# lightest/cellularautomatons3d

Hardware: AMD Instinct MI355X
Metric: Gcells/s CA step at 512^3 (higher is better)
Workload: dtype u32

## Files before the change

cellularautomatons3d_amd/csrc/ca3d_api.cpp:

```cpp
#include <cstdarg>
#include <cstdio>
#include <cstring>
#include <cstdlib>
#include <new>
#include <stdexcept>

#include "ca3d_engine.h"

namespace
{
thread_local char g_last_error[1024] = "";
}

namespace ca3d
{
void set_last_error(const char *msg) noexcept
{
	if (!msg) msg = "";
	size_t n = strlen(msg);
	if (n >= sizeof g_last_error) n = sizeof g_last_error - 1;
	memmove(g_last_error, msg, n);
	g_last_error[n] = 0;
}

// ... 846 lines not shown
			}
			if (cur == h->cur) break;
		}
		return CA3D_OK;
	}
	if (!strcmp(name, "stats")) { h->want_stats = value ? 1 : 0; if (!value) h->ev_valid = false; return CA3D_OK; }
	if (!strcmp(name, "graph_min"))
	{
		if (value < 1 || value > kMaxGraphSteps) return fail(CA3D_ERR_INVALID_ARGUMENT, "graph_min must be in [1, %u]", kMaxGraphSteps);
		h->graph_min = (uint32_t)value;
		return CA3D_OK;
	}
	if (!strcmp(name, "render_indirect")) { h->render_indirect = value ? 1 : 0; return CA3D_OK; }
	if (!strcmp(name, "render_sched")) { h->render_sched = value ? 1 : 0; return CA3D_OK; }
	if (!strcmp(name, "render_skip")) { h->render_skip = value ? 1 : 0; return CA3D_OK; }
	if (!strcmp(name, "rows"))
	{
		h->use_rows = value ? 1 : 0;
		refresh_kernels(h);
		return CA3D_OK;
	}
	if (!strcmp(name, "render_frame_bricks")) { h->render_frame_bricks = value ? 1 : 0; return CA3D_OK; }
	if (!strcmp(name, "render_stream")) { h->render_stream = value ? 1 : 0; return CA3D_OK; }
	if (!strcmp(name, "render_pipeline"))
	{
		if (value < 0 || value > ca3d_engine::kMaxLanes) return fail(CA3D_ERR_INVALID_ARGUMENT, "render_pipeline must be 0 (off), 1 (default depth) or 2 .. %d frames in flight", ca3d_engine::kMaxLanes);
		h->render_pipeline = (int)value;
		return CA3D_OK;
	}
	if (!strcmp(name, "render_stream_check")) { h->render_stream_check = value ? 1 : 0; return CA3D_OK; }
	if (!strcmp(name, "render_row_begin") || !strcmp(name, "render_row_end"))
	{
		if (value < 0 || value > 16384) return fail(CA3D_ERR_INVALID_ARGUMENT, "row %lld is outside any target", (long long)value);
		if (name[11] == 'b')
		{
			if (value % 16) return fail(CA3D_ERR_INVALID_ARGUMENT, "render_row_begin must be a multiple of 16 (the renderer's tile height)");
			h->render_row0 = (uint32_t)value;
		}
		else h->render_row1 = (uint32_t)value;
		return CA3D_OK;
	}
	if (!strcmp(name, "render_mode"))
	{
		if (value != 0 && value != 1) return fail(CA3D_ERR_INVALID_ARGUMENT, "render_mode must be 0 (converged frame) or 1 (one literal reference frame)");
		h->render_mode = (int)value;
		return CA3D_OK;
	}
	if (!strcmp(name, "render_reset_history"))
	{
		int rc2 = bind_device(h);
		if (rc2) return rc2;
		return clear_render_history(h);
	}
	if (!strcmp(name, "fused")) { drop_graph(h); h->use_fused = value ? 1 : 0; return CA3D_OK; }
	if (!strcmp(name, "variant"))
	{
		if (value != 0 && value != 1) return fail(CA3D_ERR_INVALID_ARGUMENT, "variant must be 0 (auto) or 1 (generic kernel)");
		drop_graph(h);
		h->variant = (int)value;
		refresh_kernels(h);
		return CA3D_OK;
	}
	if (!strcmp(name, "resident"))
	{
		h->use_resident = value ? 1 : 0;
		if (value) h->res_failed = false;
		refresh_kernels(h);
		return CA3D_OK;
	}
	if (!strcmp(name, "resident_rows"))
	{
		if (value != 16 && value != 32) return fail(CA3D_ERR_INVALID_ARGUMENT, "resident_rows must be 16 or 32");
		if ((uint32_t)value != h->res_rows)
		{
			int rc2 = bind_device(h);
			if (rc2) return rc2;
			HIP_TRY(hipStreamSynchronize(h->stream));
			free_resident(h);
			h->res_rows = (uint32_t)value;
			refresh_kernels(h);
		}
		return CA3D_OK;
	}
	if (!strcmp(name, "resident_pair"))
	{
		if (value != 0 && value != 1) return fail(CA3D_ERR_INVALID_ARGUMENT, "resident_pair must be 0 or 1");
		if ((value != 0) != h->res_pair)
		{
			int rc2 = bind_device(h);
			if (rc2) return rc2;
			HIP_TRY(hipStreamSynchronize(h->stream));
			free_resident(h);
			h->res_pair = value != 0;
			refresh_kernels(h);
		}
		return CA3D_OK;
	}
	if (!strcmp(name, "resident_zsplit"))
	{
		if (value != 1 && value != 2) return fail(CA3D_ERR_INVALID_ARGUMENT, "resident_zsplit must be 1 or 2");
		h->res_zsplit = (uint32_t)value;
		refresh_kernels(h);
		return CA3D_OK;
	}
	if (!strcmp(name, "resident_min"))
	{
		if (value < 1) return fail(CA3D_ERR_INVALID_ARGUMENT, "resident_min must be >= 1");
// ... 70 lines not shown
```

cellularautomatons3d_amd/csrc/ca3d_engine.h:

```cpp
#pragma once

#include <map>
#include <string>
#include <vector>

#include "ca3d_internal.h"

struct ca3d_engine
{
	int device = 0;
	hipStream_t own_stream = nullptr;
	hipStream_t stream = nullptr;
	hipEvent_t ev_start = nullptr, ev_stop = nullptr;
	bool ev_valid = false;

	bool configured = false;
	uint32_t G = 0;
	int layout = CA3D_LAYOUT_PACKED32;
	bool slab = false;
	uint32_t z0 = 0, nz = 0, ghost = 0;
	uint32_t nplanes = 0;
	size_t plane_words = 0;
	uint32_t *buf[2] = {nullptr, nullptr};
	bool has_state = false;
	bool binary_state = false;
	uint64_t step = 0;
	uint32_t cur = 0;

	ca3d::CanonRules rules;
	int variant = 0;
	int use_graph = 1;
	int render_mode = 0;
	int render_indirect = 0;
	int render_sched = 1;
	uint32_t render_row0 = 0, render_row1 = 0;
	int use_fused = 0;

	struct StepGraph { hipGraphExec_t exec = nullptr; uint32_t launches = 0; };
	std::map<uint64_t, StepGraph> step_graphs;
	uint32_t graph_min = 128;
	int want_stats = 1;
	std::map<uint64_t, hipGraphExec_t> slab_graphs;
	uint32_t pending_edges = 0;
	bool pending_binary = true;
	bool pending_resident = false;
	int roll_z = 0;
	int roll_tile = 1;
	int use_roll = 1;
	int use_jit = 1;
	ca3d::VnJit vn_jit;
	ca3d::ClassJit class_jit;
	ca3d::RowsJit rows_jit;
	int use_rows = 1;
	ca3d::RollJit roll_jit;
	std::string jit_log;

	int use_resident = 1;
	bool res_ready = false;
	bool res_class = false;
	bool res_failed = false;
	bool res_check = false;
	void *res_jit_fn = nullptr;
	void *res_slab_fn = nullptr;
	size_t res_mail_bytes = 0;
	unsigned long long *res_mail = nullptr;
	uint32_t *res_status = nullptr, *res_status_host = nullptr;
	uint32_t res_epoch = 0;
	uint32_t res_min = 8;
	uint32_t queue_max = 0;
	uint32_t queued = 0;
	uint64_t launches_total = 0;
	bool res_pair = true;
	uint32_t res_rows = 32;
	uint32_t res_zsplit = 1;
	uint32_t res_timeout_ticks = 20000000;
	uint32_t *spare = nullptr;
	struct ResPending { uint32_t epoch0, n, cur_before; uint64_t step_before; uint32_t *in, *other, *spare; };
	std::vector<ResPending> res_pending;
	uint32_t res_fault_tile = 0;
	uint32_t res_recovered = 0;
	std::string res_note;

	void *comm = nullptr;
	int comm_rank = 0, comm_world = 0;
	hipStream_t comm_stream = nullptr;
	hipEvent_t ev_edges = nullptr, ev_comm = nullptr, ev_gather = nullptr;
	bool ghosts_valid = false;

	ca3d_stats stats{};
// ... 130 lines not shown
```

cellularautomatons3d_amd/csrc/ca3d_internal.h:

```cpp
#pragma once

#include <hip/hip_runtime.h>
#include <stdint.h>
#include <string>

#include "ca3d.h"
#include "ca_device_types.h"

namespace ca3d
{

constexpr int kMaxOffsets = 26;

struct OffsetLists
{
	uint32_t n[3];
	uint8_t code[3][32];
};

struct CanonRules
{
	bool valid = false;
	MainKind main = MAIN_GENERIC;
	bool need[3] = {false, false, false};
	bool fast = false;
	OffsetLists lists{};
	PackedRuleArgs prog{};
	uint32_t onset_survive[3]{}, onset_born[3]{};
	uint32_t unpacked_survive = 0, unpacked_born = 0;
	RuleSetProg unpacked_prog{};
	bool unpacked_fast = false;
	uint32_t survive_raw[CA3D_LUT_LEN]{}, born_raw[CA3D_LUT_LEN]{};
};

int canonicalize_rules(const int32_t *main_offs, uint32_t n_main, const int32_t *edge_offs, uint32_t n_edge,
                       const int32_t *corner_offs, uint32_t n_corner, const uint32_t *survive,
                       const uint32_t *born, CanonRules *out, std::string *err);
void compile_rule_prog(uint32_t onset_mask, uint32_t max_count, RuleProg *out);


struct VnJit
{
	void *zr1 = nullptr, *zr2 = nullptr, *zr4 = nullptr, *zr8 = nullptr;
	int cvl = -1;
	uint32_t lut_s = 0, lut_b = 0;
};

struct RowsJit
{
	void *deep = nullptr, *flat = nullptr;
	uint32_t G = 0;
	int zrun = 0, main = -1;
	bool e = false, c = false;
};

struct ClassJit
{
	void *deep = nullptr, *deep_za = nullptr, *flat = nullptr;
	void *deep_np2 = nullptr, *flat_np2 = nullptr;
	int main = -1;
	bool e = false, c = false;
};

struct RollJit
{
	void *z[3] = {nullptr, nullptr, nullptr};
	void *tile[4] = {nullptr, nullptr, nullptr, nullptr};
	void *tile_x = nullptr; int zx = 0;
	void *loop[2][2] = {{nullptr, nullptr}, {nullptr, nullptr}};
	void *w2[2] = {nullptr, nullptr};
	void *wtile[2] = {nullptr, nullptr};
	void *np2[3] = {nullptr, nullptr, nullptr};
	int cv_np2 = 0;
	int cvl = -1;
	int main = -1;
	bool e = false, c = false;
};

struct PackedLaunch
{
	const uint32_t *in;
	uint32_t *out;
	PlaneRange pr;
	const CanonRules *rules;
	int variant;
	const VnJit *vn_jit = nullptr;
	const ClassJit *class_jit = nullptr;
	const RollJit *roll_jit = nullptr;
	int roll_z = 0;
	int roll_tile = 1;
	const RowsJit *rows_jit = nullptr;
};

struct ResidentLaunch
{
// ... 147 lines not shown
	int neighbourhood;
	bool clustered;
	uint32_t first, count;
	const uint32_t *periods;
	ca3d_canon_period *out;
	uint64_t *keys;
	uint32_t keys_stride;
};
hipError_t launch_canon_period(const CanonPeriodLaunch &l, hipStream_t stream);
struct SheetLaunch
{
	const uint32_t *state;
	uint32_t first, count;
	uint32_t tile_w, tile_h, columns, spp;
	const float *uniforms;
	uint32_t *presentation;
	void *light;
	uint32_t *depth;
	unsigned long long *counters;
};
hipError_t launch_render_sheet(const SheetLaunch &l, hipStream_t stream);
uint32_t sheet_shares(uint32_t count, uint32_t blocks, uint32_t slots);
struct SeedLaunch
{
	uint32_t *buf0, *buf1;
	uint32_t G;
	int layout;
	uint32_t z0, nz, ghost;
	ca3d_seed spec;
};
hipError_t launch_seed(const SeedLaunch &l, hipStream_t stream);
hipError_t launch_seed_ensemble(uint32_t *state, uint32_t *prev, uint32_t first, uint32_t count, const ca3d_seed *specs, const ca3d_seed &one, hipStream_t stream);
const char *seed_spec_error(const ca3d_seed &s, uint32_t G);
hipError_t launch_copy_f4(const void *in, void *out, size_t bytes, hipStream_t stream);
hipError_t streams_concurrent(hipStream_t a, hipStream_t b, bool *out);
hipError_t launch_render(const RenderLaunch &l, hipStream_t stream);
size_t stream_scratch_bytes(uint32_t W, uint32_t H, uint32_t spp, size_t *hit_off, size_t *occl_off, size_t *rays_off);
size_t frame_bricks_bytes(uint32_t G);
bool frame_bricks_applies(uint32_t G);
hipError_t launch_render_frame_bricks(const void *frame_params, uint32_t *bricks, bool bricks_valid, hipStream_t stream, bool *bricks_built = nullptr);
hipError_t launch_brick_volume(const uint32_t *cells, uint32_t *bricks, uint32_t G, hipStream_t stream);
hipError_t launch_render_stream(const void *params, void *scratch, uint32_t W, uint32_t H, bool check, uint32_t *bricks, bool bricks_valid, hipStream_t stream, bool *bricks_built = nullptr, hipEvent_t before_resolve = nullptr, int walk_share_pct = 100,
                                bool *sparse_too = nullptr);

hipError_t launch_packed_step(const PackedLaunch &l, hipStream_t stream);
const char *packed_kernel_name(const CanonRules &r, uint32_t G, int variant);
bool vn_rule_applies(const CanonRules &r, int variant);
bool side_tables_silent(const CanonRules &r);
bool vn_kernel_applies(const CanonRules &r, uint32_t G, int variant);
hipError_t launch_packed_vn(const PackedLaunch &l, hipStream_t stream);
void vn_tables(const CanonRules &r, uint32_t *lut_s, uint32_t *lut_b);
bool vn_tables_prebuilt(uint32_t lut_s, uint32_t lut_b);
int vn_grid_log2(uint32_t G);
uint64_t jit_sources_hash();
int jit_vn_kernels(int device, int cvl, uint32_t lut_s, uint32_t lut_b, VnJit *out, std::string *log);
void class_tables(const CanonRules &r, uint32_t tables[6]);
int class_zrun(const CanonRules &r);
bool use_class_kernel(const CanonRules &r, uint32_t G, int variant);
int jit_class_kernels(int device, const CanonRules &r, ClassJit *out, std::string *log);
int jit_rows_kernels(int device, const CanonRules &r, uint32_t G, RowsJit *out, std::string *log);
bool rows_kernel_applies(const CanonRules &r, uint32_t G, int variant);
int jit_roll_kernels(int device, const CanonRules &r, int cvl, RollJit *out, std::string *log);
int jit_roll_np2_kernels(int device, const CanonRules &r, int cv, RollJit *out, std::string *log);
bool roll_np2_applies(const CanonRules &r, uint32_t G, int variant);
bool roll_kernel_applies(const CanonRules &r, uint32_t G, int variant);
std::string synthesize_rule_source(const CanonRules &r, int *ops_out);
std::string rule_function_source(const CanonRules &r);
bool resident_kernel_applies(const CanonRules &r, uint32_t G, int variant);
size_t resident_mail_bytes(uint32_t G, uint32_t rows);
hipError_t launch_resident(const ResidentLaunch &l, hipStream_t stream);
bool resident_capacity(uint32_t G, uint32_t rows, uint32_t zsplit, int pair, void *jit_fn, hipStream_t stream, uint32_t *tiles, uint32_t *capacity);
bool resident_slab_capacity(void *fn, hipStream_t stream, uint32_t *tiles, uint32_t *capacity);
int jit_resident_kernel(int device, uint32_t lut_s, uint32_t lut_b, uint32_t rows, uint32_t zsplit, int pair, void **fn, std::string *log);
bool resident_class_applies(const CanonRules &r, uint32_t G, int variant);
int jit_resident_class_kernel(int device, const CanonRules &r, uint32_t G, uint32_t zsplit, void **fn, std::string *log);
uint32_t resident_class_zsplit(uint32_t G);
struct ResidentSlabLaunch
{
	const uint32_t *in;
	uint32_t *out;
	unsigned long long *mail;
	uint32_t *status, *host_flag;
	uint32_t steps, epoch0, timeout_ticks;
	int dead_plane;
	void *fn;
};
int resident_slab_planes(const CanonRules &r, uint32_t G, uint32_t nplanes, int variant);
size_t resident_slab_mail_bytes();
hipError_t launch_resident_slab(const ResidentSlabLaunch &l, hipStream_t stream);
void resident_stream_retired(hipStream_t stream);
int jit_resident_slab_kernel(int device, uint32_t lut_s, uint32_t lut_b, int pz, void **fn, std::string *log);
int packed_fused_steps(const CanonRules &r, uint32_t G, int variant);
hipError_t launch_packed_fused(const PackedLaunch &l, hipStream_t stream);
hipError_t launch_unpacked_step(const UnpackedLaunch &l, hipStream_t stream, const char **kernel_name);


int exception_to_status() noexcept;
void jit_stats(ca3d_jit_stats *out);
#define CA3D_API_TRY try
#define CA3D_API_CATCH                          \
	catch (...)                                 \
	{                                           \
		return ca3d::exception_to_status();     \
	}

}
```

cellularautomatons3d_amd/csrc/ca3d_step.cpp:

```cpp
#include <cstdio>
#include <cstring>

#include "ca3d_engine.h"

namespace ca3d
{

static int submit_steps(ca3d_engine *h, uint32_t n_steps);

int enqueue_step(ca3d_engine *h, int src, uint32_t lo, uint32_t hi, hipStream_t s, bool fused, uint32_t lo2, uint32_t hi2)
{
	PlaneRange pr;
	pr.G = h->G;
	pr.nplanes = h->nplanes;
	pr.zbase = h->slab ? (int32_t)h->z0 - (int32_t)h->ghost : 0;
	pr.lo = lo;
	pr.hi = hi;
	pr.wrap_full = h->slab ? 0u : 1u;
	hipError_t e;
	if (h->layout == CA3D_LAYOUT_PACKED32)
	{
		pr.lo2 = lo2;
		pr.hi2 = hi2;
		PackedLaunch l{h->buf[src], h->buf[src ^ 1], pr, &h->rules, h->variant, h->vn_jit.cvl >= 0 ? &h->vn_jit : nullptr, h->class_jit.main >= 0 ? &h->class_jit : nullptr, (h->roll_jit.cvl >= 0 || h->roll_jit.cv_np2 > 0) ? &h->roll_jit : nullptr, h->roll_z, h->roll_tile, h->rows_jit.main >= 0 ? &h->rows_jit : nullptr};
// ... 63 lines not shown
	if (!h->use_jit) return;
	if (h->use_roll && roll_np2_applies(h->rules, h->G, h->variant))
	{
		if (hipSetDevice(h->device) != hipSuccess) return;
		RollJit rj;
		if (jit_roll_np2_kernels(h->device, h->rules, (int)(h->G / 128u), &rj, &h->jit_log) == CA3D_OK) { h->roll_jit = rj; return; }
	}
	if (h->use_rows && rows_kernel_applies(h->rules, h->G, h->variant))
	{
		if (hipSetDevice(h->device) != hipSuccess) return;
		RowsJit rj;
		if (jit_rows_kernels(h->device, h->rules, h->G, &rj, &h->jit_log) == CA3D_OK) h->rows_jit = rj;
		if (h->G == 64u && !h->res_ready && h->use_resident && !h->slab && resident_kernel_applies(h->rules, h->G, h->variant))
		{
			uint32_t ls64 = 0, lb64 = 0;
			vn_tables(h->rules, &ls64, &lb64);
			if (jit_resident_kernel(h->device, ls64, lb64, 64u, 1u, 0, &h->res_jit_fn, &h->jit_log) == CA3D_OK) h->res_ready = true;
		}
		return;
	}
	if (!vn_kernel_applies(h->rules, h->G, h->variant))
	{
		const uint32_t cv = h->G / 128u;
		if (!use_class_kernel(h->rules, h->G, h->variant) || h->G % 128u || cv > 64u) return;
		if (hipSetDevice(h->device) != hipSuccess) return;
		ClassJit cj;
		if (jit_class_kernels(h->device, h->rules, &cj, &h->jit_log) == CA3D_OK) h->class_jit = cj;
		else return;
		if (cv & (cv - 1u)) return;
		if (h->use_roll && roll_kernel_applies(h->rules, h->G, h->variant))
		{
			RollJit rj;
			if (jit_roll_kernels(h->device, h->rules, vn_grid_log2(h->G), &rj, &h->jit_log) == CA3D_OK) h->roll_jit = rj;
		}
		if (h->use_resident && !h->slab && resident_class_applies(h->rules, h->G, h->variant) &&
		    jit_resident_class_kernel(h->device, h->rules, h->G, resident_class_zsplit(h->G), &h->res_jit_fn, &h->jit_log) == CA3D_OK)
		{
			h->res_ready = true;
			h->res_class = true;
		}
		return;
	}
	uint32_t ls = 0, lb = 0;
	vn_tables(h->rules, &ls, &lb);
	const bool resident = h->use_resident && !h->slab && resident_kernel_applies(h->rules, h->G, h->variant);
	if (vn_tables_prebuilt(ls, lb)) return;
	if (hipSetDevice(h->device) != hipSuccess) return;
	VnJit j;
	if (jit_vn_kernels(h->device, vn_grid_log2(h->G), ls, lb, &j, &h->jit_log) == CA3D_OK) h->vn_jit = j;
	const ResidentShape shape = resident_shape(h);
	if (resident && jit_resident_kernel(h->device, ls, lb, h->G == 256u ? 256u : shape.rows, shape.zsplit, shape.pair, &h->res_jit_fn, &h->jit_log) == CA3D_OK) h->res_ready = true;
}

void reported_kernel_name(const ca3d_engine *h, char *out, size_t n_bytes)
{
	const char *name = "";
	const bool fused = h->configured && h->rules.valid && h->layout == CA3D_LAYOUT_PACKED32 && h->use_fused && !h->slab && packed_fused_steps(h->rules, h->G, h->variant) == 2;
	if (h->configured && h->rules.valid)
	{
		if (h->layout != CA3D_LAYOUT_PACKED32) name = h->step > 0 && h->unpacked_kernel[0] ? h->unpacked_kernel : "ca_unpacked";
		else if (fused) name = "ca_packed_fused+ca_packed_class";
		else if (resident_enabled(h)) name = h->res_class ? "ca_resident_class(jit)" : (h->res_jit_fn ? "ca_resident_vn(jit)" : "ca_resident_vn");
		else if (h->slab && resident_slab_enabled(h)) name = "ca_resident_slab_vn(jit)";
		else if (h->roll_jit.cv_np2 > 0) name = "ca_packed_roll_np2(jit)";
		else if (h->rows_jit.main >= 0) name = "ca_packed_rows(jit)";
		else name = h->vn_jit.cvl >= 0 ? "ca_packed_vn(jit)" : packed_kernel_name(h->rules, h->G, h->variant);
	}
	const bool class_jit = h->configured && h->rules.valid && h->layout == CA3D_LAYOUT_PACKED32 && h->class_jit.main >= 0 && strncmp(name, "ca_resident", 11) != 0 && !fused;
	if (class_jit && h->roll_jit.cvl >= 0 && !strncmp(name, "ca_packed_class", 15))
		snprintf(out, n_bytes, "ca_packed_class_roll%s(jit)", name + 15);
	else
		snprintf(out, n_bytes, "%s%s", name, class_jit ? "(jit)" : "");
}

static void check_residency(ca3d_engine *h)
{
	h->res_note.clear();
	if (!h->res_ready && !h->res_slab_fn) return;
	if (hipSetDevice(h->device) != hipSuccess) return;
	uint32_t tiles = 0, cap = 0;
	char buf[256];
	if (h->res_ready)
	{
		const ResidentShape shape = resident_shape(h);
		if (resident_capacity(h->G, shape.rows, shape.zsplit, shape.pair, h->res_jit_fn, h->stream, &tiles, &cap) && cap < tiles)
		{
			h->res_ready = false;
			h->res_class = false;
			snprintf(buf, sizeof buf, "resident multi-step kernel not selected: it needs %u co-resident workgroups, this device / stream holds %u; per-step kernels in use", tiles, cap);
			h->res_note = buf;
		}
	}
	if (h->res_slab_fn && resident_slab_capacity(h->res_slab_fn, h->stream, &tiles, &cap) && cap < tiles)
	{
		h->res_slab_fn = nullptr;
		snprintf(buf, sizeof buf, "resident slab kernel not selected: it needs %u co-resident workgroups, this device / stream holds %u; per-step kernels in use", tiles, cap);
		h->res_note = buf;
	}
}

static void note_jit_failure(const ca3d_engine *h)
{
	if (!h->jit_log.empty()) fail(0, "run-time kernel specialisation failed, pre-built kernels in use: %s", h->jit_log.c_str());
	else if (!h->res_note.empty()) set_last_error(h->res_note.c_str());
}

void refresh_kernels(ca3d_engine *h)
{
	select_kernels(h);
	check_residency(h);
	note_jit_failure(h);
}

constexpr size_t kMaxStepGraphs = 24;

static void plan_steps(const ca3d_engine *h, uint32_t n, uint32_t *n_fused, uint32_t *n_single)
{
	uint32_t f = 0;
	if (h->use_fused && h->layout == CA3D_LAYOUT_PACKED32 && !h->slab && packed_fused_steps(h->rules, h->G, h->variant) == 2 && n >= 3)
	{
		f = (n - 1u) / 2u;
		f &= ~1u;
	}
	*n_fused = f;
	*n_single = n - 2u * f;
}

static int enqueue_batch(ca3d_engine *h, uint32_t n, uint32_t start_buf, hipStream_t s, uint64_t *launches)
{
	uint32_t f, single;
	plan_steps(h, n, &f, &single);
	uint32_t cur = start_buf;
	for (uint32_t i = 0; i < f; i++, cur ^= 1u)
	{
		int rc = enqueue_step(h, (int)cur, 0, h->G, s, true);
		if (rc) return rc;
	}
	for (uint32_t i = 0; i < single; i++, cur ^= 1u)
	{
		int rc = enqueue_step(h, (int)cur, 0, h->G, s, false);
		if (rc) return rc;
	}
	if (launches) *launches += f + single;
	return CA3D_OK;
}

int step_graph(ca3d_engine *h, uint32_t n, uint32_t start, ca3d_engine::StepGraph **out)
{
	const uint64_t key = ((uint64_t)start << 32) | n;
	auto it = h->step_graphs.find(key);
	if (it != h->step_graphs.end()) { *out = &it->second; return CA3D_OK; }
	if (h->step_graphs.size() >= kMaxStepGraphs)
	{
		HIP_TRY(hipStreamSynchronize(h->stream));
		for (auto &kv : h->step_graphs) hipGraphExecDestroy(kv.second.exec);
		h->step_graphs.clear();
	}
	uint64_t launches = 0;
	ca3d_engine::StepGraph g;
	int rc = capture_graph(h, [&]() { return enqueue_batch(h, n, start, h->stream, &launches); }, &g.exec);
	if (rc) return rc;
	g.launches = (uint32_t)launches;
	*out = &h->step_graphs.emplace(key, g).first->second;
	return CA3D_OK;
}

int check_resident(ca3d_engine *h)
{
	if (!h->res_status_host) return CA3D_OK;
	if (!h->res_check && h->res_pending.empty()) return CA3D_OK;
	h->res_check = false;
	if (*h->res_status_host == 0) { h->res_pending.clear(); return CA3D_OK; }
// ... 252 lines not shown
```

cellularautomatons3d_amd/csrc/ca_jit.cpp:

```cpp
#include <hip/hip_runtime.h>
#include <hip/hiprtc.h>

#include <sys/stat.h>
#include <unistd.h>

#include <cerrno>
#include <chrono>
#include <cstdio>
#include <cstdlib>
#include <cstring>
#include <map>
#include <mutex>
#include <string>
#include <vector>

#include "ca3d_internal.h"
#include "ca_jit_sources.h"

namespace ca3d
{
namespace
{
std::mutex g_mutex;
std::map<std::string, hipModule_t> g_modules;
// ... 357 lines not shown
}

int jit_roll_kernels(int device, const CanonRules &r, int cvl, RollJit *out, std::string *log)
{
	std::lock_guard<std::mutex> lock(g_mutex);
	std::string key = "roll/" + std::to_string(device) + "/" + std::to_string(cvl) + "/";
	std::vector<std::string> defines = {"-DCA3D_JIT_CVL=" + std::to_string(cvl)};
	add_rule(r, &key, &defines);
	const int zx = getenv("CA3D_ROLL_ZX") ? atoi(getenv("CA3D_ROLL_ZX")) : 0;
	if (zx > 0)
	{
		key += "/zx" + std::to_string(zx);
		defines.push_back("-DCA3D_ROLL_ZX=" + std::to_string(zx));
	}
	hipModule_t mod = nullptr;
	int rc = build_module(key, "ca3d_jit_roll.hip", kSrc_ca_jit_prog_roll, defines, &mod, log, rule_function_source(r));
	if (!rc) rc = get_entries(mod, {{"ca3d_jit_roll_z2", &out->z[0]}, {"ca3d_jit_roll_z4", &out->z[1]}, {"ca3d_jit_roll_z8", &out->z[2]},
	                                {"ca3d_jit_tile_z2", &out->tile[0]}, {"ca3d_jit_tile_z4", &out->tile[1]}, {"ca3d_jit_tile_z8", &out->tile[2]}, {"ca3d_jit_tile_z16", &out->tile[3]},
	                                {"ca3d_jit_rloop_z15", &out->loop[0][0]}, {"ca3d_jit_rloop_z30", &out->loop[0][1]}, {"ca3d_jit_tloop_z15", &out->loop[1][0]}, {"ca3d_jit_tloop_z30", &out->loop[1][1]}}, log);
	if (!rc && cvl <= 4) rc = get_entries(mod, {{"ca3d_jit_roll2_z8", &out->w2[0]}, {"ca3d_jit_roll2_z16", &out->w2[1]}}, log);
	if (!rc && cvl <= 5) rc = get_entries(mod, {{"ca3d_jit_wtile_z8", &out->wtile[0]}, {"ca3d_jit_wtile_z16", &out->wtile[1]}}, log);
	if (!rc && zx > 0) rc = get_entries(mod, {{"ca3d_jit_tile_zx", &out->tile_x}}, log);
	if (rc) return rc;
	out->zx = zx > 0 ? zx : 0;
	out->cvl = cvl;
	out->main = (int)r.main;
	out->e = r.need[1];
	out->c = r.need[2];
	return CA3D_OK;
}

uint64_t jit_sources_hash()
{
	static const uint64_t h = [] {
		uint64_t x = 1469598103934665603ull;
		auto add = [&x](const char *src) { for (const char *c = src; c && *c; c++) { x ^= (unsigned char)*c; x *= 1099511628211ull; } };
		for (const auto &hd : kJitHeaders) add(hd.text);
		add(getenv("CA3D_JIT_FLAGS"));
		return x;
	}();
	return h;
}

int jit_vn_kernels(int device, int cvl, uint32_t lut_s, uint32_t lut_b, VnJit *out, std::string *log)
{
	std::lock_guard<std::mutex> lock(g_mutex);
	const std::string key = "vn/" + std::to_string(device) + "/" + std::to_string(cvl) + "/" + std::to_string(lut_s) + "/" + std::to_string(lut_b);
	const std::vector<std::string> defines = {"-DCA3D_JIT_CVL=" + std::to_string(cvl), "-DCA3D_JIT_LS=" + std::to_string(lut_s & 0xFFu),
	                                          "-DCA3D_JIT_LB=" + std::to_string(lut_b & 0xFFu)};
	hipModule_t mod = nullptr;
	int rc = build_module(key, "ca3d_jit_vn.hip", kSrc_ca_jit_prog_vn, defines, &mod, log);
	if (!rc) rc = get_entries(mod, {{"ca3d_jit_vn_zr1", &out->zr1}, {"ca3d_jit_vn_zr2", &out->zr2}, {"ca3d_jit_vn_zr4", &out->zr4}}, log);
	if (!rc && cvl >= 4) rc = get_entries(mod, {{"ca3d_jit_vn_zr8", &out->zr8, false}}, log);
	if (rc) return rc;
	out->cvl = cvl;
	out->lut_s = lut_s;
	out->lut_b = lut_b;
	return CA3D_OK;
}

void jit_stats(ca3d_jit_stats *out)
{
	std::lock_guard<std::mutex> lock(g_mutex);
	*out = g_stats;
	const std::string &d = cache_dir();
	memset(out->cache_dir, 0, sizeof out->cache_dir);
	strncpy(out->cache_dir, d.c_str(), sizeof out->cache_dir - 1);
}

}
```

cellularautomatons3d_amd/csrc/ca_jit_prog_vn.inc:

```
namespace ca3d_jit
{
#include "ca_bitops.inc"
#include "ca_packed_vn_kernel.inc"
}
```

cellularautomatons3d_amd/csrc/ca_packed.hip:

```cpp
#include <algorithm>
#include <cstdlib>

#include "ca3d_internal.h"

namespace ca3d
{
namespace
{

#include "ca_bitslice.inc"

#include "ca_packed_class_kernel.inc"

struct RollArgs
{
	u32 lo, hi, nplanes, wrap_full;
	u32 lo2, hi2, runs1;
	int zbase;
};

struct FusedGeom
{
	u32 LPR, lpr_shift;
	u32 nstrips;
// ... 423 lines not shown
	if (!use_class_kernel(r, G, variant) || vn_kernel_applies(r, G, variant)) return false;
	const uint32_t cv = G / 128u;
	if (G % 128u || (cv & (cv - 1u)) || cv < 2u || cv > 64u) return false;
	const bool diagonals_or_z = r.need[1] || r.need[2] || r.main == MAIN_MOORE || r.main == MAIN_EDGES || r.main == MAIN_CORNERS || r.main == MAIN_VN;
	return diagonals_or_z;
}

bool roll_np2_applies(const CanonRules &r, uint32_t G, int variant)
{
	static const int env = getenv("CA3D_ROLL_NP2") ? atoi(getenv("CA3D_ROLL_NP2")) : 1;
	if (!env || variant == 1 || !r.fast || G % 128u) return false;
	const uint32_t cv = G / 128u;
	if ((cv & (cv - 1u)) == 0 || cv < 3u || cv > 7u) return false;
	return r.need[1] || r.need[2] || r.main == MAIN_MOORE || r.main == MAIN_EDGES || r.main == MAIN_CORNERS || r.main == MAIN_VN;
}

int class_zrun(const CanonRules &r)
{
	const bool diagonals = r.need[1] || r.need[2] || r.main == MAIN_MOORE || r.main == MAIN_EDGES || r.main == MAIN_CORNERS;
	return diagonals ? 4 : 2;
}

bool rows_kernel_applies(const CanonRules &r, uint32_t G, int variant)
{
	if (variant == 1 || !r.fast || G % 32u || G < 32u || G > 2048u) return false;
	const uint32_t cv = G / 128u;
	const bool p2_uint4 = G % 128u == 0 && (cv & (cv - 1u)) == 0;
	if (p2_uint4) return false;
	static const int np2_env = getenv("CA3D_ROWS_NP2") ? atoi(getenv("CA3D_ROWS_NP2")) : -1;
	if (G % 128u == 0) return np2_env >= 0 ? np2_env != 0 : (class_zrun(r) == 4 || G < 768u);
	return true;
}

bool use_class_kernel(const CanonRules &r, uint32_t G, int variant)
{
	return variant != 1 && r.fast && ((G / 32u) % 4u) == 0;
}


const char *packed_kernel_name(const CanonRules &r, uint32_t G, int variant)
{
	if (vn_kernel_applies(r, G, variant)) return "ca_packed_vn";
	if (!use_class_kernel(r, G, variant)) return "ca_packed_generic";
	static const char *names[6][4] = {
	    {"ca_packed_class<vn>", "ca_packed_class<vn,E>", "ca_packed_class<vn,C>", "ca_packed_class<vn,E,C>"},
	    {"ca_packed_class<vn2d>", "ca_packed_class<vn2d,E>", "ca_packed_class<vn2d,C>", "ca_packed_class<vn2d,E,C>"},
	    {"ca_packed_class<moore>", "ca_packed_class<moore,E>", "ca_packed_class<moore,C>", "ca_packed_class<moore,E,C>"},
	    {"ca_packed_class<moore2d>", "ca_packed_class<moore2d,E>", "ca_packed_class<moore2d,C>", "ca_packed_class<moore2d,E,C>"},
	    {"ca_packed_class<edges>", "ca_packed_class<edges,E>", "ca_packed_class<edges,C>", "ca_packed_class<edges,E,C>"},
	    {"ca_packed_class<corners>", "ca_packed_class<corners,E>", "ca_packed_class<corners,C>", "ca_packed_class<corners,E,C>"}};
	return names[r.main][(r.need[1] ? 1 : 0) + (r.need[2] ? 2 : 0)];
}

int packed_fused_steps(const CanonRules &r, uint32_t G, int variant)
{
	FusedGeom g;
	int W;
	if (variant != 0 || !use_class_kernel(r, G, variant)) return 0;
	if (r.main != MAIN_VN && r.main != MAIN_VN2D) return 0;
	if (r.need[1] || r.need[2]) return 0;
	return fused_geometry(G, &g, &W) ? 2 : 0;
}

hipError_t launch_packed_fused(const PackedLaunch &l, hipStream_t stream)
{
	if (l.pr.hi <= l.pr.lo) return hipSuccess;
	switch (l.rules->main)
	{
	case MAIN_VN: return launch_fused<MAIN_VN, false, false>(l, stream);
	case MAIN_VN2D: return launch_fused<MAIN_VN2D, false, false>(l, stream);
	default: return hipErrorInvalidValue;
	}
}

hipError_t launch_packed_step(const PackedLaunch &l, hipStream_t stream)
{
	const CanonRules &r = *l.rules;
	if (l.pr.hi <= l.pr.lo)
	{
		if (l.pr.hi2 <= l.pr.lo2) return hipSuccess;
		PackedLaunch only = l;
		only.pr.lo = l.pr.lo2; only.pr.hi = l.pr.hi2; only.pr.lo2 = only.pr.hi2 = 0;
		return launch_packed_step(only, stream);
	}
	if (vn_kernel_applies(r, l.pr.G, l.variant)) return launch_packed_vn(l, stream);
	if (const RollJit *rj = l.roll_jit; rj && rj->cv_np2 > 0 && (u32)rj->cv_np2 * 128u == l.pr.G && rj->main == (int)r.main && rj->e == r.need[1] && rj->c == r.need[2])
	{
		const bool two = l.pr.hi2 > l.pr.lo2;
		const u32 G = l.pr.G, CV = G / 128u, R = 64u / CV, bpp = ((G + R - 1u) / R + 3u) / 4u;
		const u32 planes1 = l.pr.hi - l.pr.lo, planes2 = two ? l.pr.hi2 - l.pr.lo2 : 0u;
		const u32 shortest = two ? (planes1 < planes2 ? planes1 : planes2) : planes1;
		for (int zi = 2; zi >= 0; zi--)
		{
			const u32 Z = 2u << zi;
			if (shortest < Z || !rj->np2[zi]) continue;
			const u32 runs1 = (planes1 + Z - 1u) / Z, nruns = runs1 + (planes2 + Z - 1u) / Z;
			if (l.roll_z ? l.roll_z != (int)Z : (zi > 0 && (size_t)bpp * nruns < 512u)) continue;
			RollArgs a;
			a.lo = l.pr.lo; a.hi = l.pr.hi; a.nplanes = l.pr.nplanes; a.wrap_full = l.pr.wrap_full; a.zbase = l.pr.zbase;
			a.lo2 = l.pr.lo2; a.hi2 = two ? l.pr.hi2 : l.pr.lo2; a.runs1 = runs1;
			const u32 *in = l.in;
			u32 *out = l.out;
			void *args[] = {(void *)&in, (void *)&out, (void *)&a};
			return hipModuleLaunchKernel((hipFunction_t)rj->np2[zi], bpp * nruns, 1, 1, 256, 1, 1, 0, stream, args, nullptr);
		}
	}
	if (const RowsJit *rj = l.rows_jit; rj && rj->G == l.pr.G && rj->main == (int)r.main && rj->e == r.need[1] && rj->c == r.need[2] && rj->deep && rj->flat)
	{
		const bool two = l.pr.hi2 > l.pr.lo2;
		const u32 G = l.pr.G, C = G / 32u, R = C >= 64u ? 1u : 64u / C, bpp = ((G + R - 1u) / R + 3u) / 4u;
		const u32 planes1 = l.pr.hi - l.pr.lo, planes2 = two ? l.pr.hi2 - l.pr.lo2 : 0u;
		const u32 shortest = two ? (planes1 < planes2 ? planes1 : planes2) : planes1;
		const u32 Z = shortest >= (u32)rj->zrun && (size_t)bpp * ((planes1 + planes2) / (u32)rj->zrun) >= 1024u ? (u32)rj->zrun : 1u;
		RowsArgs a;
		a.runs1 = (planes1 + Z - 1u) / Z;
		a.nt = (size_t)l.pr.nplanes * G * C * sizeof(u32) <= (16u << 20) ? 1u : 0u;
		const u32 nruns = a.runs1 + (planes2 + Z - 1u) / Z;
		const u32 *in = l.in;
		u32 *out = l.out;
// ... 35 lines not shown
```

cellularautomatons3d_amd/csrc/ca_packed_vn.hip:

```cpp
#include <hip/hip_runtime.h>
#include <stdint.h>

#include "ca3d_internal.h"

namespace ca3d
{
namespace
{
#include "ca_bitops.inc"

#include "ca_packed_vn_kernel.inc"

constexpr int kDefaultS = 0xFF, kDefaultB = 0x0A;

template <int CVL, int ZR>
hipError_t launch(const PackedLaunch &l, VnArgs a, hipStream_t stream)
{
	a.runs1 = (l.pr.hi - l.pr.lo + ZR - 1u) / ZR;
	constexpr u32 CV = 1u << CVL, TPP = 128u * CV * CV / 256u;
	const u32 blocks = TPP * (a.runs1 + (l.pr.hi2 > l.pr.lo2 ? (l.pr.hi2 - l.pr.lo2 + ZR - 1u) / ZR : 0u));
	static const int order_env = getenv("CA3D_VN_ORDER") ? atoi(getenv("CA3D_VN_ORDER")) : 0;
	const bool one_range = !(l.pr.hi2 > l.pr.lo2) && (l.pr.hi - l.pr.lo) % ZR == 0;
	a.zfast = one_range && a.runs1 % 8u == 0 && order_env == 1 ? a.runs1 / 8u : 0u;
	const VnJit *jit = l.vn_jit;
	if (a.lut_s == (u32)kDefaultS && a.lut_b == (u32)kDefaultB)
		hipLaunchKernelGGL((ca_packed_vn<CVL, ZR, kDefaultS, kDefaultB>), dim3(blocks), dim3(256), 0, stream, l.in, l.out, a);
	else if (void *fn = ZR == 1 ? (jit ? jit->zr1 : nullptr) : ZR == 2 ? (jit ? jit->zr2 : nullptr) : ZR == 4 ? (jit ? jit->zr4 : nullptr) : (jit ? jit->zr8 : nullptr);
	         fn && jit->cvl == CVL && jit->lut_s == a.lut_s && jit->lut_b == a.lut_b)
	{
		const u32 *in = l.in;
		u32 *out = l.out;
		void *args[] = {(void *)&in, (void *)&out, (void *)&a};
		return hipModuleLaunchKernel((hipFunction_t)fn, blocks, 1, 1, 256, 1, 1, 0, stream, args, nullptr);
	}
	else
		hipLaunchKernelGGL((ca_packed_vn<CVL, ZR, -1, -1>), dim3(blocks), dim3(256), 0, stream, l.in, l.out, a);
	return hipGetLastError();
}

int log2_exact(u32 x)
{
	if (!x || (x & (x - 1u))) return -1;
	int s = 0;
	while ((1u << s) < x) s++;
	return s;
}

}

bool side_tables_silent(const CanonRules &r)
{
	if (!r.fast) return false;
	for (int s = 1; s < 3; s++)
	{
		const uint32_t reachable = (2u << r.lists.n[s]) - 1u;
		if ((r.onset_born[s] | r.onset_survive[s]) & reachable) return false;
	}
	return true;
}

bool vn_rule_applies(const CanonRules &r, int variant) { return variant != 1 && r.main == MAIN_VN && side_tables_silent(r); }

bool vn_kernel_applies(const CanonRules &r, uint32_t G, int variant)
{
	if (!vn_rule_applies(r, variant)) return false;
	const int cvl = log2_exact(G / 128u);
	return G % 128u == 0 && cvl >= 1 && cvl <= 6;
}

void vn_tables(const CanonRules &r, uint32_t *lut_s, uint32_t *lut_b)
{
	*lut_s = r.onset_survive[0] & 0x7Fu;
	*lut_b = r.onset_born[0] & 0x7Fu;
	if ((*lut_s & 0x2Au) == 0x2Au) *lut_s |= 0x80u;
	if ((*lut_b & 0x2Au) == 0x2Au) *lut_b |= 0x80u;
}

bool vn_tables_prebuilt(uint32_t lut_s, uint32_t lut_b) { return lut_s == (u32)kDefaultS && lut_b == (u32)kDefaultB; }

int vn_grid_log2(uint32_t G) { return log2_exact(G / 128u); }

hipError_t launch_packed_vn(const PackedLaunch &l, hipStream_t stream)
{
	const CanonRules &r = *l.rules;
	const bool two = l.pr.hi2 > l.pr.lo2;
	const u32 G = l.pr.G, planes = l.pr.hi - l.pr.lo + (two ? l.pr.hi2 - l.pr.lo2 : 0u);
	const u32 shortest = two ? (l.pr.hi - l.pr.lo < l.pr.hi2 - l.pr.lo2 ? l.pr.hi - l.pr.lo : l.pr.hi2 - l.pr.lo2) : l.pr.hi - l.pr.lo;
	const int cvl = log2_exact(G / 128u);
	VnArgs a;
	a.lo = l.pr.lo; a.hi = l.pr.hi; a.nplanes = l.pr.nplanes; a.wrap_full = l.pr.wrap_full; a.zbase = l.pr.zbase;
	a.lo2 = l.pr.lo2; a.hi2 = two ? l.pr.hi2 : l.pr.lo2; a.runs1 = 0;
	vn_tables(r, &a.lut_s, &a.lut_b);
	a.nt = (size_t)l.pr.nplanes * G * (G / 32u) * sizeof(u32) <= (16u << 20) ? 1u : 0u;
	static const int zr_env = getenv("CA3D_VN_ZR") ? atoi(getenv("CA3D_VN_ZR")) : 0;
	const u32 tpp = G / 128u * G / 256u;
	const bool deep = shortest >= 2u && (size_t)tpp * ((planes + 1u) / 2u) >= 1024u;
	const bool deep4 = zr_env != 2 && cvl >= 4 && shortest >= 4u && (size_t)tpp * ((planes + 3u) / 4u) >= 4096u;
	const bool prebuilt = a.lut_s == (u32)kDefaultS && a.lut_b == (u32)kDefaultB;
	const bool has8 = prebuilt || (l.vn_jit && l.vn_jit->zr8 && l.vn_jit->cvl == cvl && l.vn_jit->lut_s == a.lut_s && l.vn_jit->lut_b == a.lut_b);
	const bool deep8 = zr_env != 2 && zr_env != 4 && cvl >= 4 && has8 && shortest >= 8u && (size_t)tpp * ((planes + 7u) / 8u) >= 4096u;
	if (deep8) return cvl == 4 ? launch<4, 8>(l, a, stream) : cvl == 5 ? launch<5, 8>(l, a, stream) : launch<6, 8>(l, a, stream);
	switch (cvl)
	{
	case 1: return launch<1, 1>(l, a, stream);
	case 2: return deep ? launch<2, 2>(l, a, stream) : launch<2, 1>(l, a, stream);
	case 3: return deep ? launch<3, 2>(l, a, stream) : launch<3, 1>(l, a, stream);
	case 4: return deep4 ? launch<4, 4>(l, a, stream) : deep ? launch<4, 2>(l, a, stream) : launch<4, 1>(l, a, stream);
	case 5: return deep4 ? launch<5, 4>(l, a, stream) : deep ? launch<5, 2>(l, a, stream) : launch<5, 1>(l, a, stream);
	case 6: return deep4 ? launch<6, 4>(l, a, stream) : deep ? launch<6, 2>(l, a, stream) : launch<6, 1>(l, a, stream);
	default: return hipErrorInvalidValue;
	}
}

}
```

Before: 58780.

## Add two-step fused VN kernel with LDS halo exchange, auto-enabled for large grids

Result: slower. 57880 (-1.5%).

```diff
diff --git a/cellularautomatons3d_amd/csrc/ca3d_api.cpp b/cellularautomatons3d_amd/csrc/ca3d_api.cpp
--- a/cellularautomatons3d_amd/csrc/ca3d_api.cpp
+++ b/cellularautomatons3d_amd/csrc/ca3d_api.cpp
@@ -922,7 +922,7 @@
 		if (rc2) return rc2;
 		return clear_render_history(h);
 	}
-	if (!strcmp(name, "fused")) { drop_graph(h); h->use_fused = value ? 1 : 0; return CA3D_OK; }
+	if (!strcmp(name, "fused")) { drop_graph(h); h->use_fused = value < 0 ? -1 : (value ? 1 : 0); return CA3D_OK; }
 	if (!strcmp(name, "variant"))
 	{
 		if (value != 0 && value != 1) return fail(CA3D_ERR_INVALID_ARGUMENT, "variant must be 0 (auto) or 1 (generic kernel)");
diff --git a/cellularautomatons3d_amd/csrc/ca3d_engine.h b/cellularautomatons3d_amd/csrc/ca3d_engine.h
--- a/cellularautomatons3d_amd/csrc/ca3d_engine.h
+++ b/cellularautomatons3d_amd/csrc/ca3d_engine.h
@@ -34,7 +34,7 @@
 	int render_indirect = 0;
 	int render_sched = 1;
 	uint32_t render_row0 = 0, render_row1 = 0;
-	int use_fused = 0;
+	int use_fused = -1;
 
 	struct StepGraph { hipGraphExec_t exec = nullptr; uint32_t launches = 0; };
 	std::map<uint64_t, StepGraph> step_graphs;
diff --git a/cellularautomatons3d_amd/csrc/ca3d_internal.h b/cellularautomatons3d_amd/csrc/ca3d_internal.h
--- a/cellularautomatons3d_amd/csrc/ca3d_internal.h
+++ b/cellularautomatons3d_amd/csrc/ca3d_internal.h
@@ -41,6 +41,7 @@
 
 struct VnJit
 {
+	void *vn2 = nullptr;
 	void *zr1 = nullptr, *zr2 = nullptr, *zr4 = nullptr, *zr8 = nullptr;
 	int cvl = -1;
 	uint32_t lut_s = 0, lut_b = 0;
@@ -294,6 +295,13 @@
 void vn_tables(const CanonRules &r, uint32_t *lut_s, uint32_t *lut_b);
 bool vn_tables_prebuilt(uint32_t lut_s, uint32_t lut_b);
 int vn_grid_log2(uint32_t G);
+struct Vn2Geometry
+{
+	uint32_t G, threads, strip_rows, run_planes;
+};
+Vn2Geometry vn2_geometry(uint32_t G);
+bool vn2_available(uint32_t lut_s, uint32_t lut_b, int cvl, const VnJit *jit);
+hipError_t launch_packed_vn2(const PackedLaunch &l, hipStream_t stream);
 uint64_t jit_sources_hash();
 int jit_vn_kernels(int device, int cvl, uint32_t lut_s, uint32_t lut_b, VnJit *out, std::string *log);
 void class_tables(const CanonRules &r, uint32_t tables[6]);
@@ -333,6 +341,7 @@
 void resident_stream_retired(hipStream_t stream);
 int jit_resident_slab_kernel(int device, uint32_t lut_s, uint32_t lut_b, int pz, void **fn, std::string *log);
 int packed_fused_steps(const CanonRules &r, uint32_t G, int variant);
+bool packed_fused_generic_applies(const CanonRules &r, uint32_t G, int variant);
 hipError_t launch_packed_fused(const PackedLaunch &l, hipStream_t stream);
 hipError_t launch_unpacked_step(const UnpackedLaunch &l, hipStream_t stream, const char **kernel_name);
 
diff --git a/cellularautomatons3d_amd/csrc/ca3d_step.cpp b/cellularautomatons3d_amd/csrc/ca3d_step.cpp
--- a/cellularautomatons3d_amd/csrc/ca3d_step.cpp
+++ b/cellularautomatons3d_amd/csrc/ca3d_step.cpp
@@ -139,13 +139,33 @@
 	if (resident && jit_resident_kernel(h->device, ls, lb, h->G == 256u ? 256u : shape.rows, shape.zsplit, shape.pair, &h->res_jit_fn, &h->jit_log) == CA3D_OK) h->res_ready = true;
 }
 
+constexpr size_t kFusedAutoMinBufferBytes = (size_t)128 << 20;
+
+static int fused_form(const ca3d_engine *h)
+{
+	if (!h->configured || !h->rules.valid || h->layout != CA3D_LAYOUT_PACKED32 || h->slab || !h->use_fused) return 0;
+	if (packed_fused_steps(h->rules, h->G, h->variant) != 2) return 0;
+	int form = 1;
+	if (vn_kernel_applies(h->rules, h->G, h->variant))
+	{
+		uint32_t ls = 0, lb = 0;
+		vn_tables(h->rules, &ls, &lb);
+		if (vn2_available(ls, lb, vn_grid_log2(h->G), h->vn_jit.cvl >= 0 ? &h->vn_jit : nullptr)) form = 2;
+		else if (!packed_fused_generic_applies(h->rules, h->G, h->variant)) return 0;
+	}
+	if (h->use_fused < 0 && !(form == 2 && h->buffer_words() * sizeof(uint32_t) >= kFusedAutoMinBufferBytes)) return 0;
+	return form;
+}
+
 void reported_kernel_name(const ca3d_engine *h, char *out, size_t n_bytes)
 {
 	const char *name = "";
-	const bool fused = h->configured && h->rules.valid && h->layout == CA3D_LAYOUT_PACKED32 && h->use_fused && !h->slab && packed_fused_steps(h->rules, h->G, h->variant) == 2;
+	const int form = fused_form(h);
+	const bool fused = form != 0;
 	if (h->configured && h->rules.valid)
 	{
 		if (h->layout != CA3D_LAYOUT_PACKED32) name = h->step > 0 && h->unpacked_kernel[0] ? h->unpacked_kernel : "ca_unpacked";
+		else if (form == 2) name = h->vn_jit.cvl >= 0 ? "ca_packed_vn2+ca_packed_vn(jit)" : "ca_packed_vn2+ca_packed_vn";
 		else if (fused) name = "ca_packed_fused+ca_packed_class";
 		else if (resident_enabled(h)) name = h->res_class ? "ca_resident_class(jit)" : (h->res_jit_fn ? "ca_resident_vn(jit)" : "ca_resident_vn");
 		else if (h->slab && resident_slab_enabled(h)) name = "ca_resident_slab_vn(jit)";
@@ -204,7 +224,7 @@
 static void plan_steps(const ca3d_engine *h, uint32_t n, uint32_t *n_fused, uint32_t *n_single)
 {
 	uint32_t f = 0;
-	if (h->use_fused && h->layout == CA3D_LAYOUT_PACKED32 && !h->slab && packed_fused_steps(h->rules, h->G, h->variant) == 2 && n >= 3)
+	if (n >= 3 && fused_form(h))
 	{
 		f = (n - 1u) / 2u;
 		f &= ~1u;
diff --git a/cellularautomatons3d_amd/csrc/ca_jit.cpp b/cellularautomatons3d_amd/csrc/ca_jit.cpp
--- a/cellularautomatons3d_amd/csrc/ca_jit.cpp
+++ b/cellularautomatons3d_amd/csrc/ca_jit.cpp
@@ -433,6 +433,7 @@
 	int rc = build_module(key, "ca3d_jit_vn.hip", kSrc_ca_jit_prog_vn, defines, &mod, log);
 	if (!rc) rc = get_entries(mod, {{"ca3d_jit_vn_zr1", &out->zr1}, {"ca3d_jit_vn_zr2", &out->zr2}, {"ca3d_jit_vn_zr4", &out->zr4}}, log);
 	if (!rc && cvl >= 4) rc = get_entries(mod, {{"ca3d_jit_vn_zr8", &out->zr8, false}}, log);
+	if (!rc) rc = get_entries(mod, {{"ca3d_jit_vn2", &out->vn2}}, log);
 	if (rc) return rc;
 	out->cvl = cvl;
 	out->lut_s = lut_s;
diff --git a/cellularautomatons3d_amd/csrc/ca_jit_prog_vn.inc b/cellularautomatons3d_amd/csrc/ca_jit_prog_vn.inc
--- a/cellularautomatons3d_amd/csrc/ca_jit_prog_vn.inc
+++ b/cellularautomatons3d_amd/csrc/ca_jit_prog_vn.inc
@@ -2,4 +2,5 @@
 {
 #include "ca_bitops.inc"
 #include "ca_packed_vn_kernel.inc"
+#include "ca_packed_vn2_kernel.inc"
 }
diff --git a/cellularautomatons3d_amd/csrc/ca_packed.hip b/cellularautomatons3d_amd/csrc/ca_packed.hip
--- a/cellularautomatons3d_amd/csrc/ca_packed.hip
+++ b/cellularautomatons3d_amd/csrc/ca_packed.hip
@@ -499,19 +499,31 @@
 	return names[r.main][(r.need[1] ? 1 : 0) + (r.need[2] ? 2 : 0)];
 }
 
-int packed_fused_steps(const CanonRules &r, uint32_t G, int variant)
+bool packed_fused_generic_applies(const CanonRules &r, uint32_t G, int variant)
 {
 	FusedGeom g;
 	int W;
-	if (variant != 0 || !use_class_kernel(r, G, variant)) return 0;
-	if (r.main != MAIN_VN && r.main != MAIN_VN2D) return 0;
-	if (r.need[1] || r.need[2]) return 0;
-	return fused_geometry(G, &g, &W) ? 2 : 0;
+	if (variant != 0 || !use_class_kernel(r, G, variant)) return false;
+	if (r.main != MAIN_VN && r.main != MAIN_VN2D) return false;
+	if (r.need[1] || r.need[2]) return false;
+	return fused_geometry(G, &g, &W);
+}
+
+int packed_fused_steps(const CanonRules &r, uint32_t G, int variant)
+{
+	return vn_kernel_applies(r, G, variant) || packed_fused_generic_applies(r, G, variant) ? 2 : 0;
 }
 
 hipError_t launch_packed_fused(const PackedLaunch &l, hipStream_t stream)
 {
 	if (l.pr.hi <= l.pr.lo) return hipSuccess;
+	if (vn_kernel_applies(*l.rules, l.pr.G, l.variant))
+	{
+		uint32_t ls = 0, lb = 0;
+		vn_tables(*l.rules, &ls, &lb);
+		if (vn2_available(ls, lb, vn_grid_log2(l.pr.G), l.vn_jit)) return launch_packed_vn2(l, stream);
+		if (!packed_fused_generic_applies(*l.rules, l.pr.G, l.variant)) return hipErrorInvalidValue;
+	}
 	switch (l.rules->main)
 	{
 	case MAIN_VN: return launch_fused<MAIN_VN, false, false>(l, stream);
diff --git a/cellularautomatons3d_amd/csrc/ca_packed_vn.hip b/cellularautomatons3d_amd/csrc/ca_packed_vn.hip
--- a/cellularautomatons3d_amd/csrc/ca_packed_vn.hip
+++ b/cellularautomatons3d_amd/csrc/ca_packed_vn.hip
@@ -10,6 +10,7 @@
 #include "ca_bitops.inc"
 
 #include "ca_packed_vn_kernel.inc"
+#include "ca_packed_vn2_kernel.inc"
 
 constexpr int kDefaultS = 0xFF, kDefaultB = 0x0A;
 
@@ -36,6 +37,32 @@
 	else
 		hipLaunchKernelGGL((ca_packed_vn<CVL, ZR, -1, -1>), dim3(blocks), dim3(256), 0, stream, l.in, l.out, a);
 	return hipGetLastError();
+}
+
+constexpr int vn2_ntl(int cvl) { return cvl <= 3 ? 8 : cvl == 4 ? 9 : 10; }
+constexpr int kVn2Ahead = 2;
+
+template <int CVL>
+hipError_t launch_vn2(const PackedLaunch &l, u32 lut_s, u32 lut_b, hipStream_t stream)
+{
+	constexpr int NTL = vn2_ntl(CVL);
+	const Vn2Geometry g = vn2_geometry(128u << CVL);
+	Vn2Args a;
+	a.zl = g.run_planes;
+	a.groups = (g.run_planes + 2u) / 6u;
+	a.nstrips = (g.G + g.strip_rows - 3u) / (g.strip_rows - 2u);
+	const u32 blocks = a.nstrips * ((g.G + a.zl - 1u) / a.zl);
+	if (lut_s == (u32)kDefaultS && lut_b == (u32)kDefaultB)
+	{
+		hipLaunchKernelGGL((ca_packed_vn2<CVL, NTL, kVn2Ahead, kDefaultS, kDefaultB>), dim3(blocks), dim3(1u << NTL), 0, stream, l.in, l.out, a);
+		return hipGetLastError();
+	}
+	const VnJit *jit = l.vn_jit;
+	if (!jit || !jit->vn2 || jit->cvl != CVL || jit->lut_s != lut_s || jit->lut_b != lut_b) return hipErrorInvalidValue;
+	const u32 *in = l.in;
+	u32 *out = l.out;
+	void *args[] = {(void *)&in, (void *)&out, (void *)&a};
+	return hipModuleLaunchKernel((hipFunction_t)jit->vn2, blocks, 1, 1, 1u << NTL, 1, 1, 0, stream, args, nullptr);
 }
 
 int log2_exact(u32 x)
@@ -80,6 +107,46 @@
 
 int vn_grid_log2(uint32_t G) { return log2_exact(G / 128u); }
 
+Vn2Geometry vn2_geometry(uint32_t G)
+{
+	const int cvl = log2_exact(G / 128u);
+	Vn2Geometry g;
+	g.G = G;
+	g.threads = 1u << vn2_ntl(cvl);
+	g.strip_rows = vn2_strip_rows(cvl, vn2_ntl(cvl));
+	static const int zl_env = getenv("CA3D_VN2_ZL") ? atoi(getenv("CA3D_VN2_ZL")) : 0;
+	u32 zl = 16u;
+	const u32 nstrips = (G + g.strip_rows - 3u) / (g.strip_rows - 2u), per_cu = 1024u / g.threads;
+	for (u32 z : {64u, 34u, 28u})
+		if ((size_t)nstrips * ((G + z - 1u) / z) >= 2u * 256u * per_cu) { zl = z; break; }
+	if (zl_env >= 4 && (u32)zl_env <= G && (zl_env + 2) % 6 == 0) zl = (u32)zl_env;
+	g.run_planes = zl;
+	return g;
+}
+
+bool vn2_available(uint32_t lut_s, uint32_t lut_b, int cvl, const VnJit *jit)
+{
+	if (vn_tables_prebuilt(lut_s, lut_b)) return true;
+	return jit && jit->vn2 && jit->cvl == cvl && jit->lut_s == lut_s && jit->lut_b == lut_b;
+}
+
+hipError_t launch_packed_vn2(const PackedLaunch &l, hipStream_t stream)
+{
+	if (l.pr.lo != 0 || l.pr.hi != l.pr.G || l.pr.hi2 > l.pr.lo2 || !l.pr.wrap_full || l.pr.nplanes != l.pr.G) return hipErrorInvalidValue;
+	u32 ls, lb;
+	vn_tables(*l.rules, &ls, &lb);
+	switch (log2_exact(l.pr.G / 128u))
+	{
+	case 1: return launch_vn2<1>(l, ls, lb, stream);
+	case 2: return launch_vn2<2>(l, ls, lb, stream);
+	case 3: return launch_vn2<3>(l, ls, lb, stream);
+	case 4: return launch_vn2<4>(l, ls, lb, stream);
+	case 5: return launch_vn2<5>(l, ls, lb, stream);
+	case 6: return launch_vn2<6>(l, ls, lb, stream);
+	default: return hipErrorInvalidValue;
+	}
+}
+
 hipError_t launch_packed_vn(const PackedLaunch &l, hipStream_t stream)
 {
 	const CanonRules &r = *l.rules;
diff --git a/cellularautomatons3d_amd/csrc/ca_packed_vn2_kernel.inc b/cellularautomatons3d_amd/csrc/ca_packed_vn2_kernel.inc
--- /dev/null
+++ b/cellularautomatons3d_amd/csrc/ca_packed_vn2_kernel.inc
@@ -0,0 +1,168 @@
+
+struct Vn2Args
+{
+	u32 zl;
+	u32 groups;
+	u32 nstrips;
+};
+
+constexpr u32 vn2_strip_rows(int cvl, int ntl) { return (1u << ntl) >> cvl; }
+
+template <int CVL, int LS, int LB>
+__device__ __forceinline__ uint4 vn2_words(const uint4 &c, const uint4 &m, const uint4 &p, const uint4 &b, const uint4 &a, u32 lomask, bool last, int lane)
+{
+	const u32 w[4] = {c.x, c.y, c.z, c.w};
+	const u32 wm[4] = {m.x, m.y, m.z, m.w};
+	const u32 wp[4] = {p.x, p.y, p.z, p.w};
+	const u32 wb[4] = {b.x, b.y, b.z, b.w};
+	const u32 wa[4] = {a.x, a.y, a.z, a.w};
+	const u32 lo = dpp_mov<kDppWaveShr1>(w[3]) & lomask;
+	const u32 nxt = dpp_mov<kDppWaveShl1>(w[0]);
+	const u32 first = row_first<CVL>(w[0], lane);
+	const u32 hi = CVL == 6 ? first : (last ? first : nxt);
+	u32 o[4];
+#pragma unroll
+	for (int i = 0; i < 4; i++)
+	{
+		const u32 l = from_left(w[i], i ? w[i > 0 ? i - 1 : 0] : lo);
+		const u32 r = from_right(i < 3 ? w[i < 3 ? i + 1 : 0] : hi, w[i]);
+		o[i] = vn_next<LS, LB>(w[i], l, r, wp[i], wm[i], wa[i], wb[i]);
+	}
+	return make_uint4(o[0], o[1], o[2], o[3]);
+}
+
+template <int CVL, int NTL, int AHEAD, int LS, int LB>
+__device__ __forceinline__ void vn2_run(const u32 *__restrict__ in, u32 *__restrict__ out, const Vn2Args &a, uint4 *lds)
+{
+	static_assert(LS >= 0 && LB >= 0, "the two-step kernel exists for compile-time tables only");
+	static_assert(AHEAD >= 1 && AHEAD <= 4, "load-ahead depth");
+	constexpr u32 CV = 1u << CVL;
+	constexpr int G = 128 << CVL;
+	constexpr u32 NT = 1u << NTL;
+	constexpr int S = (int)vn2_strip_rows(CVL, NTL), SO = S - 2;
+	static_assert(S >= 4 && SO <= G, "strip height");
+	constexpr u32 ROW_BYTES = CV * 16u, PLANE_BYTES = (u32)G * ROW_BYTES;
+
+	const u32 bi = blockIdx.x, nb = gridDim.x;
+	const u32 v = (nb & 7u) == 0 ? (bi & 7u) * (nb >> 3) + (bi >> 3) : bi;
+	const u32 run = v / a.nstrips, strip = v - run * a.nstrips;
+	const int zl = (int)a.zl;
+	const int y0 = min((int)strip * SO, G - SO);
+	const int z0 = min((int)run * zl, G - zl);
+
+	const u32 tid = threadIdx.x;
+	const int lane = (int)(tid & 63u);
+	const int r = (int)(tid >> CVL);
+	const u32 cxv = tid & (CV - 1u);
+	const int gy = y0 - 1 + r;
+	const int gyw = gy < 0 ? 0 : (gy & (G - 1));
+	const u32 oc = ((u32)gyw * CV + cxv) * 16u;
+	const u32 om = (u32)max((int)oc - (int)ROW_BYTES, 0);
+	const u32 op = (oc + ROW_BYTES) & (PLANE_BYTES - 1u);
+
+	u32 ymask = gyw == 0 ? 0u : 0xFFFFFFFFu;
+	u32 rowlive = gy < 0 ? 0u : 0xFFFFFFFFu;
+	u32 lomask = cxv == 0 ? 0u : 0xFFFFFFFFu;
+	asm volatile("" : "+v"(ymask), "+v"(rowlive), "+v"(lomask));
+	const bool last = cxv == CV - 1u;
+	const bool wave_has_row0 = __builtin_amdgcn_ballot_w64(gyw == 0) != 0;
+	const bool wave_has_dead = __builtin_amdgcn_ballot_w64(gy < 0) != 0;
+	const bool store_row = r >= 1 && r <= S - 2;
+	const u32 lds_m = (u32)max((int)tid - (int)CV, 0), lds_p = min(tid + CV, NT - 1u);
+
+	const int qmax = z0 + zl + 1;
+	auto plane = [&](int q) -> const char * {
+		q = min(q, qmax);
+		const int qa = q < 0 ? 0 : (q >= G ? q - G : q);
+		return reinterpret_cast<const char *>(in) + (size_t)qa * PLANE_BYTES;
+	};
+
+	uint4 cb = *reinterpret_cast<const uint4 *>(plane(z0 - 2) + oc);
+	uint4 cc = *reinterpret_cast<const uint4 *>(plane(z0 - 1) + oc);
+	uint4 ga[AHEAD], gm[AHEAD], gp[AHEAD];
+#pragma unroll
+	for (int k = 0; k < AHEAD; k++)
+	{
+		ga[k] = *reinterpret_cast<const uint4 *>(plane(z0 + k) + oc);
+		const char *pl = plane(z0 - 1 + k);
+		gm[k] = *reinterpret_cast<const uint4 *>(pl + om);
+		gp[k] = *reinterpret_cast<const uint4 *>(pl + op);
+	}
+	const uint4 zero4 = make_uint4(0u, 0u, 0u, 0u);
+	uint4 g1b = zero4, g1c = zero4, ym1 = zero4, yp1 = zero4;
+	char *dst = reinterpret_cast<char *>(out) + oc;
+
+	for (u32 grp = 0; grp < a.groups; grp++)
+	{
+#pragma unroll
+		for (int k = 0; k < 6; k++)
+		{
+			const int i = (int)grp * 6 + k, P = z0 - 1 + i;
+			const uint4 na = *reinterpret_cast<const uint4 *>(plane(P + 1 + AHEAD) + oc);
+			const char *pl = plane(P + AHEAD);
+			const uint4 nm = *reinterpret_cast<const uint4 *>(pl + om);
+			const uint4 np = *reinterpret_cast<const uint4 *>(pl + op);
+			__builtin_amdgcn_sched_barrier(0);
+
+			const uint4 ca = ga[0];
+			uint4 wm = gm[0], wb = cb;
+			const uint4 wp = gp[0];
+			if (__builtin_expect(wave_has_row0, 0))
+			{
+				asm volatile("");
+				wm.x &= ymask; wm.y &= ymask; wm.z &= ymask; wm.w &= ymask;
+			}
+			if (__builtin_expect((P & (G - 1)) == 0, 0))
+			{
+				asm volatile("");
+				wb = zero4;
+			}
+			uint4 g1a = vn2_words<CVL, LS, LB>(cc, wm, wp, wb, ca, lomask, last, lane);
+			if (__builtin_expect(P < 0, 0))
+			{
+				asm volatile("");
+				g1a = zero4;
+			}
+			if (__builtin_expect(wave_has_dead, 0))
+			{
+				asm volatile("");
+				g1a.x &= rowlive; g1a.y &= rowlive; g1a.z &= rowlive; g1a.w &= rowlive;
+			}
+			uint4 *slot = lds + (size_t)(i & 1) * NT;
+			slot[tid] = g1a;
+			__syncthreads();
+			const uint4 ymn = slot[lds_m], ypn = slot[lds_p];
+
+			const uint4 res = vn2_words<CVL, LS, LB>(g1c, ym1, yp1, g1b, g1a, lomask, last, lane);
+			if (i >= 2 && store_row) *reinterpret_cast<uint4 *>(dst + (size_t)(P - 1) * PLANE_BYTES) = res;
+
+			cb = cc; cc = ca;
+			g1b = g1c; g1c = g1a;
+			ym1 = ymn; yp1 = ypn;
+#pragma unroll
+			for (int q = 0; q + 1 < AHEAD; q++) { ga[q] = ga[q + 1]; gm[q] = gm[q + 1]; gp[q] = gp[q + 1]; }
+			ga[AHEAD - 1] = na; gm[AHEAD - 1] = nm; gp[AHEAD - 1] = np;
+		}
+	}
+}
+
+#ifdef CA3D_JIT
+#ifndef CA3D_JIT_VN2_NTL
+#define CA3D_JIT_VN2_NTL (CA3D_JIT_CVL <= 3 ? 8 : CA3D_JIT_CVL == 4 ? 9 : 10)
+#endif
+#ifndef CA3D_JIT_VN2_AHEAD
+#define CA3D_JIT_VN2_AHEAD 2
+#endif
+extern "C" __global__ __launch_bounds__(1 << (CA3D_JIT_VN2_NTL)) void ca3d_jit_vn2(const u32 *__restrict__ in, u32 *__restrict__ out, Vn2Args a)
+{
+	__shared__ uint4 lds[2u << (CA3D_JIT_VN2_NTL)];
+	vn2_run<CA3D_JIT_CVL, (CA3D_JIT_VN2_NTL), CA3D_JIT_VN2_AHEAD, CA3D_JIT_LS, CA3D_JIT_LB>(in, out, a, lds);
+}
+#else
+template <int CVL, int NTL, int AHEAD, int LS, int LB>
+__global__ __launch_bounds__(1 << NTL) void ca_packed_vn2(const u32 *__restrict__ in, u32 *__restrict__ out, Vn2Args a)
+{
+	__shared__ uint4 lds[2u << NTL];
+	vn2_run<CVL, NTL, AHEAD, LS, LB>(in, out, a, lds);
+}
+#endif
```
